# marzer/rt

Hardware: AMD Instinct MI355X
Metric: Mrays/s (W*H*spp per second) and wall-clock, 1920x1080x256spp scenes/basic.toml (higher is better)
Workload: dtype f32

## Files before the change

### rt_amd/csrc/context.hip

```cpp
#include "internal.hpp"

#include <algorithm>
#include <exception>
#include <new>

using namespace rt_hip;

namespace rt_hip
{
	namespace
	{
		thread_local std::string g_last_error;
	}

	rt_hip_status fail(rt_hip_status status, const char* format, ...)
	{
		char buffer[512];
		va_list args;
		va_start(args, format);
		std::vsnprintf(buffer, sizeof(buffer), format, args);
		va_end(args);
		g_last_error = buffer;
		return status;
	}
// ... 29 lines not shown
	return ok();
}

extern "C" rt_hip_status rt_hip_create(rt_hip_ctx** out_ctx, int device)
{
	if (!out_ctx)
		return fail(RT_HIP_INVALID_ARGUMENT, "rt_hip_create: out_ctx is NULL");
	*out_ctx = nullptr;
	int count = 0;
	if (hipGetDeviceCount(&count) != hipSuccess || count <= 0)
		return fail(RT_HIP_NO_DEVICE, "rt_hip_create: no HIP device is visible");
	if (device < 0 || device >= count)
		return fail(RT_HIP_NO_DEVICE, "rt_hip_create: device %d out of range (%d visible)", device, count);
	RT_HIP_TRY(hipSetDevice(device));
	hipDeviceProp_t props{};
	RT_HIP_TRY(hipGetDeviceProperties(&props, device));
	if (std::strncmp(props.gcnArchName, "gfx950", 6) != 0)
		return fail(RT_HIP_NO_DEVICE, "rt_hip_create: device %d is %s; this module is built for gfx950 only", device, props.gcnArchName);

	rt_hip_ctx* ctx = new (std::nothrow) rt_hip_ctx;
	if (!ctx)
		return fail(RT_HIP_RUNTIME_ERROR, "rt_hip_create: out of host memory");
	ctx->device = device;
	ctx->compute_units = props.multiProcessorCount > 0 ? static_cast<uint32_t>(props.multiProcessorCount) : 256u;
	ctx->workgroup_lds_bytes = props.sharedMemPerBlock;
	ctx->numa_node = numa_node_of(device);
	if (const char* knob = std::getenv("RT_HIP_NUMA_NODE"))
	{
		char* end = nullptr;
		const long v = std::strtol(knob, &end, 10);
		if (end != knob && v >= -1 && v < 1024)
			ctx->numa_node = static_cast<int>(v);
	}
	hipError_t e = ctx->counters.reserve(sizeof(device_counters));
	if (e == hipSuccess)
		e = hipEventCreate(&ctx->render_begin);
	if (e == hipSuccess)
		e = hipEventCreate(&ctx->render_end);
	if (e == hipSuccess)
		e = hipEventCreateWithFlags(&ctx->stripes_ready, hipEventDisableTiming);
	if (e == hipSuccess)
		e = hipEventCreateWithFlags(&ctx->counters_copied, hipEventDisableTiming);
	if (e == hipSuccess)
		e = hipEventCreate(&ctx->gathered);
	if (e == hipSuccess)
		e = hipEventCreate(&ctx->assembled);
	if (e == hipSuccess)
		e = hipEventCreate(&ctx->copied);
	if (e == hipSuccess)
		e = hipHostMalloc(reinterpret_cast<void**>(&ctx->counters_host), sizeof(device_counters), hipHostMallocDefault);
	if (e == hipSuccess)
		e = hipStreamCreateWithFlags(&ctx->stream, hipStreamNonBlocking);
	if (e != hipSuccess)
	{
		rt_hip_destroy(ctx);
		return fail(RT_HIP_RUNTIME_ERROR, "rt_hip_create: %s", hipGetErrorString(e));
	}
	*out_ctx = ctx;
	return ok();
}

extern "C" rt_hip_status rt_hip_create_multi(rt_hip_ctx** out_ctx, const int* devices, int n_devices, uint32_t multi_flags)
{
	if (!out_ctx)
		return fail(RT_HIP_INVALID_ARGUMENT, "rt_hip_create_multi: out_ctx is NULL");
	*out_ctx = nullptr;
// ... 401 lines not shown
```

### rt_amd/csrc/internal.hpp

```cpp
#pragma once

#include "../../include/rt_hip.h"
#include "contract.hpp"
#include "delivery.hpp"
#include "frame_group.hpp"
#include "kernels.hpp"
#include "progressive.hpp"
#include "adaptive.hpp"
#include "lights.hpp"

#include <rccl/rccl.h>

#include <atomic>
#include <chrono>
#include <condition_variable>
#include <cstdarg>
#include <cstdio>
#include <cstdlib>
#include <cstring>
#include <memory>
#include <mutex>
#include <string>
#include <thread>
#include <vector>

namespace rt_hip
{
	rt_hip_status fail(rt_hip_status status, const char* format, ...) __attribute__((format(printf, 2, 3)));
	const std::string& last_error();
	inline rt_hip_status ok() { return RT_HIP_OK; }

#define RT_HIP_TRY_NCCL(expr)                                                                                          \
	do                                                                                                                 \
	{                                                                                                                  \
		const ncclResult_t rt_hip_try_res = (expr);                                                                    \
		if (rt_hip_try_res != ncclSuccess)                                                                             \
			return ::rt_hip::fail(RT_HIP_RUNTIME_ERROR, "%s failed: %s", #expr, ncclGetErrorString(rt_hip_try_res));   \
	}                                                                                                                  \
	while (false)

#define RT_HIP_TRY(expr)                                                                                               \
	do                                                                                                                 \
// ... 219 lines not shown
	uint32_t box_bvh_count = 0;
	bool box_bvh_built = false;
	uint64_t box_bvh_sphere_stamp = 0;
	uint64_t box_bvh_builds = 0;
	size_t scene_bytes = 0;
	std::vector<float> emission;
	bool have_emission = false;
	uint32_t emission_rows = 0, emission_lights = 0;
	uint64_t emission_version = 0;
	rt_hip::device_buffer light_tables;
	uint64_t light_tables_uploads = 0, light_tables_version = 0;
	const float4* light_shading = nullptr;
	const uint32_t* light_scatter = nullptr;
	const float4* light_shading_sm = nullptr;
	const uint32_t* light_scatter_sm = nullptr;
	void* pinned_frame = nullptr;
	size_t pinned_bytes = 0;
	void* refused_frame = nullptr;
	size_t refused_bytes = 0;

	const void* asked_pointer = nullptr;
	bool asked_pointer_is_host = false;

	rt_hip_stats stats{};

	rt_hip::pass_state progressive;
	uint32_t progressive_passes = 0;
	rt_hip::device_buffer accum;
	std::vector<uint32_t> progressive_frame;
	rt_hip::denoise_state denoise;
	rt_hip::temporal_state temporal;
	rt_hip::adaptive_accumulation adaptive;

	rt_hip_ctx() = default;
	rt_hip_ctx(const rt_hip_ctx&) = delete;
	rt_hip_ctx& operator=(const rt_hip_ctx&) = delete;
};

namespace rt_hip
{
	rt_hip_ctx* member_of(rt_hip_ctx* ctx, int rank);

	struct scene_layout
	{
		size_t scx, scy, scz, sr, sm;
		size_t pnx, pny, pnz, pd, pm;
		size_t shading, type;
		size_t geometry, prim_shading, prim_metal;
		size_t prim_shading_sm, prim_scatter_sm;
		size_t box_bounds, albedo;
		size_t total;
	};
	struct scene_request
	{
		const rt_hip_scene* scene = nullptr;
		scene_layout layout{};
		uint64_t print = 0;
		bool indices_checked = false;
		const unsigned char* image = nullptr;
		small_scene small{}, small_sm{};
	};
	rt_hip_status open_request(scene_request& r, const rt_hip_scene* scene);
	rt_hip_status make_resident(rt_hip_ctx* ctx, scene_request& r);
	rt_hip_status ensure_bvh(rt_hip_ctx* ctx, bool device_build, hipStream_t stream, bool wait);
	rt_hip_status ensure_box_bvh(rt_hip_ctx* ctx, hipStream_t stream);
	rt_hip_status ensure_light_tables(rt_hip_ctx* ctx);

	struct render_pass
	{
		uint32_t first_sample, n_samples;
		float* d_accum;
		bool adaptive = false;
	};
	rt_hip_status render_device(rt_hip_ctx* ctx, uint32_t width, uint32_t height, uint64_t seed, uint32_t flags, const rt_hip_partition* part, uint32_t* d_rgba8, float* d_rgb_f32, void* stream, bool whole_frame_buffers, bool keep_stats, bool host_frame,
								const render_pass* pass = nullptr);
	rt_hip_status fetch_member_stats(rt_hip_ctx* ctx);
	rt_hip_stats stats_of_group_rank(const rt_hip_ctx* ctx, uint32_t rank);
	void sum_group_stats(const rt_hip_ctx* ctx, rt_hip_stats* out);

	constexpr uint32_t max_frame_side = 1u << 15;
	const char* refused_guide_flag(uint32_t flags);
	bool buffers_overlap(const void* a, size_t a_bytes, const void* b, size_t b_bytes);
	frame_params centre_frame_params(uint32_t width, uint32_t height, const float* matrix);
	rt_hip_status launch_guide(rt_hip_ctx* ctx, uint32_t width, uint32_t height, const float* matrix, bool trace_boxes, float* d_guide, hipStream_t stream);
	rt_hip_status launch_filter(rt_hip_ctx* ctx, uint32_t width, uint32_t height, const float* d_in, const float* d_guide, const rt_hip_denoise_params& params, float* d_out, uint32_t* d_rgba, hipStream_t stream);

	rt_hip_status render_multi(rt_hip_ctx* root, const rt_hip_scene* scene, uint32_t* pixels_rgba8888, uint32_t width, uint32_t height, uint64_t seed, uint32_t flags, float* rgb_f32, rt_hip_stats* stats, std::chrono::steady_clock::time_point entered);
	rt_hip_status render_group(rt_hip_ctx* ctx, const rt_hip_scene* scene, uint32_t* pixels_rgba8888, uint32_t width, uint32_t height, uint64_t seed, uint32_t flags, float* rgb_f32, rt_hip_stats* stats, std::chrono::steady_clock::time_point entered);

	int numa_node_of(int device);
	bool debug_frame();
	void place_stripes(void* ptr, size_t bytes, uint32_t width, uint32_t height, uint32_t stripe_rows, const std::vector<int>& node_of_rank);
	void unpin_frame(rt_hip_ctx* ctx);
	void track_frame_buffer(rt_hip_ctx* ctx, uint32_t* pixels, size_t bytes, bool pin, bool may_move_pages = true, const std::vector<int>* stripe_nodes = nullptr, uint32_t width = 0, uint32_t height = 0);
	uint32_t live_frame_locks();

	struct staging_frame
	{
		void* ptr = nullptr;
		size_t bytes = 0;
		bool registered = false;
		int view_device = -1;
		void* view = nullptr;
		hipError_t reserve(size_t wanted, int numa_node);
		void release();
		~staging_frame() { release(); }
		template <typename T>
		T* as() const
// ... 49 lines not shown
```

### rt_amd/csrc/kernels.hip

```cpp
#include "kernels.hpp"
#include "contract.hpp"
#include "scan.hpp"
#include "bvh_scan.hpp"
#include "box_bvh_scan.hpp"
#include "scan_streamed.hpp"
#include "handover.hpp"
#include "pixel_output.hpp"
#include "lane_state.hpp"
#include "queue_build.hpp"
#include "camera_forms.hpp"

#ifdef RT_HIP_FAST_BUILD
#define render_queue render_queue_fast
#define launch_render launch_render_fast
#endif

#include "../../include/rt_hip.h"

#include <algorithm>

#ifdef RT_HIP_REGION_COUNTERS
#define RT_HIP_REGION(i)                                                                                               \
	do                                                                                                                 \
	{                                                                                                                  \
// ... 54 lines not shown
			else if (RESIDENT)
			{
				for (uint32_t i = threadIdx.x; i < lds_spheres + s.n_planes; i += block_threads)
					lds[i] = s.primitive_geometry[(s.n_spheres - lds_spheres) + i];
			}
			if constexpr (BOXES && !BOXTREE)
			{
				for (uint32_t i = threadIdx.x; i < 2u * s.n_boxes; i += block_threads)
					lds_boxes[i] = s.box_bounds[i];
			}
			__syncthreads();

#ifdef RT_HIP_REGION_COUNTERS
			uint32_t region_runs[device_counters::regions] = {}, region_lanes[device_counters::regions] = {};
#endif
			const queue_words words = unpack_words<build>(q, item_sums, pixel_done);
			const uint32_t first_chunk = PASS ? words.first_chunk : 0u;
			float* const accum = PASS ? words.accum : nullptr;
			device_bvh bvh{};
			if constexpr (BVH)
				bvh = *words.bvh;
			device_box_bvh box_tree{};
			if constexpr (BOXTREE)
				box_tree = *words.box_tree;
			const uint32_t lane = threadIdx.x & 63u;
			const uint32_t wave = threadIdx.x >> 6;
			const uint32_t chunk_items = q.chunks << q.pixels_log2;
			const uint32_t items = HALF ? 2u * chunk_items : chunk_items;
			float* const slots = reinterpret_cast<float*>(lds + table_float4s) + static_cast<size_t>(wave) * chunk_items * slot_floats;
			const uint32_t tile_w = 1u << q.tile_w_log2;
			const uint32_t tile_h = (1u << q.pixels_log2) >> q.tile_w_log2;

			const uint32_t tile_x0 = (blockIdx.x * 4u + wave) * tile_w;
			const uint32_t tile_y0 = (gridDim.y - 1u - blockIdx.y) * tile_h;
			uint32_t next_item = 0;
			unsigned long long tile_stopped = 0;
			float* pass_sums = nullptr;
			if constexpr (ADAPT)
			{
				const adaptive_words adaptive = unpack_adaptive_words(accum, p);
				pass_sums = adaptive.pass_sums;
				const uint32_t lx = tile_x0 + (lane & (tile_w - 1u));
				const uint32_t ly = tile_y0 + (lane >> q.tile_w_log2);
				const bool in_frame = lane < (1u << q.pixels_log2) && lx < p.width && ly < p.local_rows;
				bool stopped = false;
				if (first_chunk && in_frame)
					stopped = (adaptive.pixel_state[static_cast<size_t>(output_row(ly, p)) * p.width + lx] & 0x80000000u) != 0u;
				tile_stopped = __builtin_amdgcn_ballot_w64(stopped);
				if ((__builtin_amdgcn_ballot_w64(in_frame) & ~tile_stopped) == 0)
					return;
			}

			const uint32_t items_per_pixel = (ROLLING && HALF) ? (p.samples_per_pixel + q.item_samples - 1u) / q.item_samples : q.chunks;
			const unsigned long long total_items = static_cast<unsigned long long>(p.width) * p.local_rows * items_per_pixel;
			unsigned long long block_next = 0, block_end = 0;
			unsigned long long prefetched = 0;
			uint32_t prefetched_count = ROLLING ? min(64u, q.lane_cap) : 64u;
			bool dry = false;
			if (ROLLING)
				prefetched = fetch_items(counters, prefetched_count);
#ifdef RT_HIP_WAVE_CLOCKS
			const unsigned long long clock_start = wall_clock64();
			unsigned long long clock_dry = 0;
#endif

			lane_state st;
			unsigned long long wave_segments = 0;
// ... 1006 lines not shown
		};

		queue_kernel select_kernel(const kernel_build& build)
		{
			if (build.scan > 0)
			{
				const int spheres = std::min(build.scan, static_cast<int>(scalar_max_spheres)), planes = std::min(build.planes, static_cast<int>(scalar_max_planes));
				for (const small_builds& known : small_kernels)
					if (known.spheres == spheres && known.planes == planes)
						return build.general_camera ? known.general_camera(build) : known.pinhole(build);
				return nullptr;
			}
			switch (build.scan)
			{
#ifndef RT_HIP_FAST_BUILD
				case scan_bvh: return table_of<scan_bvh>(build);
#endif
				case scan_resident:
					if (build.planes)
						return table_of<scan_resident, 1, false>(build);
					return build.general_camera ? table_of<scan_resident, 0, true>(build) : table_of<scan_resident, 0, false>(build);
				case scan_streamed_dense: return table_of<scan_streamed_dense>(build);
				case scan_streamed: return table_of<scan_streamed>(build);
				default: return table_of<scan_tiled>(build);
			}
		}

		struct kernel_words
		{
			queue_params queue;
			unsigned long long* item_sums;
			uint32_t* pixel_done;
		};
		kernel_words pack_words(const rolling_buffers& rolling, const launch_plan& plan)
		{
			const kernel_build& build = plan.build;
			kernel_words words = { plan.queue, rolling.item_sums, rolling.pixel_done };
			if (build.scan == scan_bvh)
				words.item_sums = reinterpret_cast<unsigned long long*>(const_cast<device_bvh*>(rolling.bvh));
#ifndef RT_HIP_FAST_BUILD
			if ((build.scan == scan_resident || build.scan == scan_bvh) && !build.boxes && !build.lights && (build.adaptive || build.pass))
			{
				words.queue.block_items = plan.first_chunk;
				words.pixel_done = reinterpret_cast<uint32_t*>(rolling.accum);
			}
#endif
			return words;
		}
	}

	uint32_t launch_render(const launch_arguments& a)
	{
		const launch_plan& plan = a.plan;
		if (plan.variant == RT_HIP_KERNEL_NONE)
			return RT_HIP_KERNEL_NONE;
		const queue_kernel kernel = select_kernel(plan.build);
		if (!kernel)
			return plan.variant;
		dim3 grid(plan.grid_x, plan.grid_y);
		if (scan_is_persistent(plan.build.scan))
		{
			launch_cache::entry& known = a.cache.persistent[plan.persistent_slot];
			if (known.lds_bytes != plan.lds_bytes || known.per_cu < 1)
			{
				int per_cu = 0;
				if (hipOccupancyMaxActiveBlocksPerMultiprocessor(&per_cu, kernel, static_cast<int>(block_threads), plan.lds_bytes) != hipSuccess || per_cu < 1)
					per_cu = 4;
				per_cu = std::min(per_cu, plan.per_cu_cap);
				(void)hipGetLastError();
				known.lds_bytes = plan.lds_bytes;
				known.per_cu = per_cu;
			}
			grid = dim3(std::min(grid.x, a.compute_units * static_cast<uint32_t>(known.per_cu)));
		}
		const kernel_words words = pack_words(a.rolling, plan);
		hipLaunchKernelGGL(kernel, grid, dim3(block_threads), plan.lds_bytes, a.stream, a.frame, words.queue, a.small, a.scene, a.scene.primitive_geometry, a.d_rgba8, a.d_rgb_f32, a.d_counters, words.item_sums, words.pixel_done);
		return plan.variant;
	}

#ifndef RT_HIP_FAST_BUILD
	void launch_preview(const frame_params& frame, const device_scene& scene, uint32_t* d_rgba8, float* d_rgb_f32, device_counters* d_counters, hipStream_t stream)
	{
		if (!frame.width || !frame.local_rows)
			return;
		const uint32_t rows_per_block = block_threads / 64u;
		const dim3 grid((frame.width + 63u) / 64u, (frame.local_rows + rows_per_block - 1u) / rows_per_block);
		hipLaunchKernelGGL(preview_frame, grid, dim3(block_threads), 0, stream, frame, scene, d_rgba8, d_rgb_f32, d_counters);
	}

	void launch_assemble(uint32_t width,
						 uint32_t height,
						 uint32_t world,
						 uint32_t stripe_rows,
						 uint32_t padded_local_rows,
						 const uint32_t* d_gathered,
						 uint32_t* d_frame,
						 uint32_t first_rank,
						 bool frame_is_host_memory,
						 hipStream_t stream)
	{
		const dim3 grid((width + block_threads - 1) / block_threads, height);
		if (frame_is_host_memory)
			hipLaunchKernelGGL(assemble_stripes<true>, grid, dim3(block_threads), 0, stream, width, height, world, stripe_rows, padded_local_rows, first_rank, d_gathered, d_frame);
		else
			hipLaunchKernelGGL(assemble_stripes<false>, grid, dim3(block_threads), 0, stream, width, height, world, stripe_rows, padded_local_rows, first_rank, d_gathered, d_frame);
	}

#endif
// ... 2 lines not shown
```

### rt_amd/csrc/kernels.hpp

```cpp
#pragma once

#include <hip/hip_runtime.h>
#include <stdint.h>
#include "launch_plan.hpp"
#include "frame_setup.hpp"

namespace rt_hip
{
	struct device_bvh
	{
		const float4* nodes;
		const float4* spheres;
		const uint32_t* order;
		const uint32_t* always;
		uint32_t root, n_tree, n_always;
		float cx, cy, cz, radius;
	};

	struct device_scene
	{
		uint32_t n_spheres, n_planes, n_materials;
		const float* sphere_cx;
		const float* sphere_cy;
		const float* sphere_cz;
// ... 51 lines not shown
#endif
#ifdef RT_HIP_BVH_CHECK
		unsigned long long bvh_checked, bvh_disagreements;
#endif
#ifdef RT_HIP_WAVE_CLOCKS
		static constexpr unsigned clocked_waves = 16384;
		unsigned long long wave_clocks[clocked_waves][3];
#endif
	};

	struct launch_cache
	{
		struct entry
		{
			size_t lds_bytes = 0;
			int per_cu = 0;
		};
		entry persistent[persistent_cache_slots];
	};

	struct launch_arguments
	{
		const frame_params& frame;
		const device_scene& scene;
		const small_scene& small;
		const launch_plan& plan;
		uint32_t* d_rgba8;
		float* d_rgb_f32;
		device_counters* d_counters;
		const rolling_buffers& rolling;
		uint32_t compute_units;
		launch_cache& cache;
		hipStream_t stream;
	};

	uint32_t launch_render(const launch_arguments& a);

	uint32_t launch_render_fast(const launch_arguments& a);

	void launch_preview(const frame_params& frame, const device_scene& scene, uint32_t* d_rgba8, float* d_rgb_f32, device_counters* d_counters, hipStream_t stream);

	void launch_assemble(uint32_t width,
						 uint32_t height,
						 uint32_t world,
						 uint32_t stripe_rows,
						 uint32_t padded_local_rows,
						 const uint32_t* d_gathered,
						 uint32_t* d_frame,
						 uint32_t first_rank,
						 bool frame_is_host_memory,
						 hipStream_t stream);
}
```

### rt_amd/csrc/render.hip

```cpp
#include "internal.hpp"

#include <algorithm>
#include <cstdio>
#include <exception>

using namespace rt_hip;

namespace
{
	bool is_host_memory(rt_hip_ctx* ctx, const void* pointer)
	{
		if (pointer != ctx->asked_pointer)
		{
			hipPointerAttribute_t attributes{};
			const hipError_t e = hipPointerGetAttributes(&attributes, pointer);
			if (e != hipSuccess)
				(void)hipGetLastError();
			ctx->asked_pointer = pointer;
			ctx->asked_pointer_is_host = e == hipSuccess && attributes.type == hipMemoryTypeHost;
		}
		return ctx->asked_pointer_is_host;
	}
}

extern "C" rt_hip_status rt_hip_render_device(rt_hip_ctx* ctx,
											  uint32_t width,
											  uint32_t height,
											  uint64_t seed,
											  uint32_t flags,
											  const rt_hip_partition* part,
											  uint32_t* d_rgba8,
											  float* d_rgb_f32,
											  void* stream)
{
	return render_device(ctx, width, height, seed, flags, part, d_rgba8, d_rgb_f32, stream, false, true, ctx && d_rgba8 && is_host_memory(ctx, d_rgba8));
}

extern "C" rt_hip_status rt_hip_render_pass_device(rt_hip_ctx* ctx,
													   uint32_t width,
													   uint32_t height,
													   uint64_t seed,
													   uint32_t flags,
													   const rt_hip_partition* part,
													   uint32_t first_sample,
													   uint32_t n_samples,
													   float* d_accum,
													   uint32_t* d_rgba8,
													   float* d_rgb_f32,
													   void* stream)
{
	if (first_sample % sample_chunk)
		return fail(RT_HIP_INVALID_ARGUMENT, "rt_hip_render_pass_device: first_sample %u is not a multiple of %u (a pass continues the chunk-wise fold of the pixel sums)", first_sample, sample_chunk);
	if (!ctx || !d_accum || !d_rgba8)
		return fail(RT_HIP_INVALID_ARGUMENT, "rt_hip_render_pass_device: NULL argument");
	if (const char* const refused = refused_pass_flag(flags))
		return fail(RT_HIP_UNSUPPORTED, "rt_hip_render_pass_device: %s is not available for passes (0x%x): they take RT_HIP_FLAG_SM_MATERIALS, RT_HIP_FLAG_BVH, RT_HIP_FLAG_BVH_DEVICE_BUILD and RT_HIP_FLAG_STATS", refused, flags);
	if (!ctx->have_scene)
		return fail(RT_HIP_NO_SCENE, "rt_hip_render_pass_device: no scene uploaded");
	const uint32_t total = ctx->samples_per_pixel;
	if (total > pass_max_samples_per_pixel)
		return fail(RT_HIP_UNSUPPORTED, "rt_hip_render_pass_device: %u samples per pixel: the samples' random windows alias beyond %u", total, pass_max_samples_per_pixel);
	if (!n_samples || first_sample >= total || n_samples > total - first_sample || (n_samples % sample_chunk && first_sample + n_samples != total))
		return fail(RT_HIP_INVALID_ARGUMENT, "rt_hip_render_pass_device: samples [%u, %u + %u) are not whole chunks of %u within the scene's %u samples per pixel (the last pass alone may end on the sample count)", first_sample,
					first_sample, n_samples, sample_chunk, total);
	const render_pass pass = { first_sample, n_samples, d_accum };
	return render_device(ctx, width, height, seed, flags & pass_flag_mask, part, d_rgba8, d_rgb_f32, stream, false, true, is_host_memory(ctx, d_rgba8), &pass);
}

namespace rt_hip
{
rt_hip_status render_device(rt_hip_ctx* ctx, uint32_t width, uint32_t height, uint64_t seed, uint32_t flags, const rt_hip_partition* part, uint32_t* d_rgba8, float* d_rgb_f32, void* stream, bool whole_frame_buffers, bool keep_stats, bool host_frame,
							const render_pass* pass)
{
	if (!ctx || !d_rgba8)
		return fail(RT_HIP_INVALID_ARGUMENT, "rt_hip_render_device: NULL argument");
	const render_check checked = check_render_request(width, height, flags, part);
	if (checked.status)
		return fail(checked.status, "%s", checked.message);
	flags = checked.flags;
	if (!ctx->have_scene)
		return fail(RT_HIP_NO_SCENE, "rt_hip_render_device: no scene uploaded");
	if (flags & RT_HIP_FLAG_EMISSION)
	{
		const light_check table = check_emission_table("rt_hip_render_device", ctx->have_emission, ctx->emission_rows, ctx->scene.n_materials);
		if (table.status)
			return fail(table.status, "%s", table.message);
	}
	RT_HIP_TRY(hipSetDevice(ctx->device));
	const hipStream_t s = static_cast<hipStream_t>(stream);
	if (ctx->launched && ctx->last_stream != s)
		RT_HIP_TRY(hipStreamSynchronize(ctx->last_stream));

	frame_request wanted{};
	wanted.width = width, wanted.height = height, wanted.partition = checked.partition;
	wanted.samples_per_pixel = pass ? pass->first_sample + pass->n_samples : ctx->samples_per_pixel, wanted.max_bounces = ctx->max_bounces;
	wanted.seed = seed, wanted.whole_frame_buffers = whole_frame_buffers;
	std::copy(ctx->inverse_view_projection, ctx->inverse_view_projection + 16, wanted.inverse_view_projection);
	const frame_params f = make_frame_params(wanted);

	launch_plan plan{};
	rolling_buffers rolling;
	if (!(flags & RT_HIP_FLAG_PREVIEW))
	{
		launch_request request{};
		request.n_spheres = ctx->scene.n_spheres, request.n_planes = ctx->scene.n_planes, request.planes_tame = ctx->scene.planes_tame != 0;
		request.width = width, request.local_rows = f.local_rows, request.samples_per_pixel = pass ? ctx->samples_per_pixel : f.samples_per_pixel;
		if (pass)
			request.pass_first_sample = pass->first_sample, request.pass_samples = pass->n_samples, request.adaptive = pass->adaptive;
		request.camera = camera_form_of(f);
		request.flags = flags, request.host_frame = host_frame, request.fast_arithmetic = (flags & RT_HIP_FLAG_FAST) != 0;
		request.n_boxes = ctx->scene.n_boxes;
		request.n_lights = (flags & RT_HIP_FLAG_EMISSION) ? ctx->emission_lights : 0u;
		request.lds_limit = ctx->workgroup_lds_bytes;
		plan = plan_launch(request);
		if (plan.refusal[0])
			return fail(RT_HIP_UNSUPPORTED, "rt_hip_render_device: %s", plan.refusal);
		if (pass && plan.slot_bytes > max_slot_bytes)
			return fail(RT_HIP_UNSUPPORTED, "rt_hip_render_pass_device: a pass of %u samples is more than the kernels hold chunk sums for (4096 per pass; the frame's samples_per_pixel has no such limit)", pass->n_samples);
		if (plan.slot_bytes > max_slot_bytes)
			return fail(RT_HIP_UNSUPPORTED, "rt_hip_render_device: %u samples per pixel are more than the kernels hold chunk sums for (4096; the reference clamps to 1000, src/scene.cpp:544)", f.samples_per_pixel);
		if (plan.build.scan == scan_bvh)
		{
			if (const rt_hip_status st = ensure_bvh(ctx, (flags & RT_HIP_FLAG_BVH) ? checked.bvh_device_build : false, s, keep_stats))
				return st;
			RT_HIP_TRY(hipSetDevice(ctx->device));
			rolling.bvh = ctx->bvh_descriptor;
		}
		if (plan.build.box_tree)
		{
			if (const rt_hip_status st = ensure_box_bvh(ctx, s))
				return st;
			rolling.bvh = ctx->box_bvh_block.as<const device_bvh>();
		}
		if (pass)
			rolling.accum = pass->d_accum;
		if (plan.build.lights)
		{
			if (const rt_hip_status st = ensure_light_tables(ctx))
				return st;
			RT_HIP_TRY(hipSetDevice(ctx->device));
		}
		if (plan.item_sums_bytes > ctx->item_sums.bytes && plan.queue.halves && plan.big_scene && ctx->item_sums.reserve(plan.item_sums_bytes) != hipSuccess)
		{
			(void)hipGetLastError();
			request.flags |= RT_HIP_FLAG_FORCE_WHOLE_CHUNKS;
			request.flags &= ~static_cast<uint32_t>(RT_HIP_FLAG_FORCE_HALF_CHUNKS);
			plan = plan_launch(request);
		}
		if (plan.item_sums_bytes > (64ull << 30))
			return fail(RT_HIP_UNSUPPORTED, "%s: %ux%u at %u samples per pixel needs %zu GiB for the chunk sums of a scene of this size", pass ? "rt_hip_render_pass_device" : "rt_hip_render_device", width, height, f.samples_per_pixel, plan.item_sums_bytes >> 30);
		if (plan.item_sums_bytes)
		{
			RT_HIP_TRY(ctx->item_sums.reserve(plan.item_sums_bytes));
			RT_HIP_TRY(ctx->pixel_done.reserve(plan.pixel_done_bytes));
			RT_HIP_TRY(hipMemsetAsync(ctx->pixel_done.ptr, 0, plan.pixel_done_bytes, s));
			rolling.item_sums = ctx->item_sums.as<unsigned long long>();
			rolling.pixel_done = ctx->pixel_done.as<uint32_t>();
		}
	}
	device_counters* const counters = ctx->counters.as<device_counters>();
	if (keep_stats)
	{
		RT_HIP_TRY(hipMemsetAsync(counters, 0, sizeof(device_counters), s));
		RT_HIP_TRY(hipEventRecord(ctx->render_begin, s));
	}
	else if (plan.big_scene)
		RT_HIP_TRY(hipMemsetAsync(&counters->next_item, 0, sizeof(counters->next_item), s));
	uint32_t variant = RT_HIP_KERNEL_PREVIEW;
	if (flags & RT_HIP_FLAG_PREVIEW)
		launch_preview(f, ctx->scene, d_rgba8, d_rgb_f32, counters, s);
	else if (flags & RT_HIP_FLAG_FAST)
		variant = launch_render_fast({ f, ctx->scene, ctx->small, plan, d_rgba8, d_rgb_f32, counters, rolling, ctx->compute_units, ctx->cache, s });
	else if (plan.build.lights)
	{
		device_scene lit = ctx->scene;
		lit.primitive_shading = ctx->light_shading, lit.primitive_scatter = ctx->light_scatter;
		lit.primitive_shading_sm = ctx->light_shading_sm, lit.primitive_scatter_sm = ctx->light_scatter_sm;
		variant = launch_render({ f, lit, (flags & RT_HIP_FLAG_SM_MATERIALS) ? ctx->small_sm : ctx->small, plan, d_rgba8, d_rgb_f32, counters, rolling, ctx->compute_units, ctx->cache, s });
	}
	else
		variant = launch_render({ f, ctx->scene, (flags & RT_HIP_FLAG_SM_MATERIALS) ? ctx->small_sm : ctx->small, plan, d_rgba8, d_rgb_f32, counters, rolling, ctx->compute_units, ctx->cache, s });
	RT_HIP_TRY(hipGetLastError());
	ctx->launched = true;
	ctx->last_stream = s;
	if (keep_stats)
	{
		RT_HIP_TRY(hipEventRecord(ctx->render_end, s));
		RT_HIP_TRY(hipMemcpyAsync(ctx->counters_host, counters, sizeof(device_counters), hipMemcpyDeviceToHost, s));
		RT_HIP_TRY(hipEventRecord(ctx->counters_copied, s));
	}
	ctx->render_recorded = keep_stats;
	ctx->stats.kernel_variant = variant;
	ctx->stats.primary_samples = static_cast<uint64_t>(f.local_rows) * width * ((flags & RT_HIP_FLAG_PREVIEW) ? 1u : (pass ? pass->n_samples : f.samples_per_pixel));
	if (!keep_stats)
	{
		ctx->stats.render_ms = 0.0f;
		ctx->stats.segments = ctx->stats.sphere_tests = ctx->stats.plane_tests = 0;
	}
	return ok();
}
}

extern "C" rt_hip_status rt_hip_assemble_device(rt_hip_ctx* ctx,
												uint32_t width,
												uint32_t height,
												uint32_t world,
												uint32_t stripe_rows,
												const uint32_t* d_gathered,
												uint32_t* d_frame,
												void* stream)
{
	if (!ctx || !d_gathered || !d_frame)
		return fail(RT_HIP_INVALID_ARGUMENT, "rt_hip_assemble_device: NULL argument");
	if (!width || !height || !world || !stripe_rows)
// ... 175 lines not shown
			return fail(RT_HIP_RUNTIME_ERROR, "rt_hip_render: out of host memory");
		struct abandon_unless_finished
		{
			frame_delivery* delivery;
			~abandon_unless_finished()
			{
				if (delivery)
					delivery->abandon();
			}
		} staged{ nullptr };
		struct drain_before_abandoning
		{
			hipStream_t stream;
			bool armed;
			~drain_before_abandoning()
			{
				if (armed && hipStreamSynchronize(stream) != hipSuccess)
					(void)hipGetLastError();
			}
		} drain{ ctx->stream, false };
		if (!d_frame)
		{
			if (const rt_hip_status st = delivery->begin(pixels_rgba8888, pixels, &d_frame))
				return st;
			staged.delivery = delivery;
		}
		const size_t rgb_bytes = pixels * 3 * sizeof(float);
		if (rgb_f32)
		{
			RT_HIP_TRY(ctx->frame_rgb.reserve(rgb_bytes));
			RT_HIP_TRY(ctx->staging_rgb.reserve(rgb_bytes));
		}
		drain.armed = true;
		if (const rt_hip_status st = render_device(ctx, width, height, seed, flags & render_flag_mask, nullptr, d_frame, rgb_f32 ? ctx->frame_rgb.as<float>() : nullptr, ctx->stream, false, keep_stats, true))
			return st;
		if (staged.delivery)
			staged.delivery->launched();
		hipError_t e = hipSuccess;
		if (rgb_f32)
			e = hipMemcpyAsync(ctx->staging_rgb.ptr, ctx->frame_rgb.ptr, rgb_bytes, hipMemcpyDeviceToHost, ctx->stream);
		const auto issued = std::chrono::steady_clock::now();
		if (e == hipSuccess && keep_stats)
			e = hipEventSynchronize(ctx->render_end);
		const auto t0 = std::chrono::steady_clock::now();
		const hipError_t drained = hipStreamSynchronize(ctx->stream);
		drain.armed = drained != hipSuccess;
		RT_HIP_TRY(e);
		RT_HIP_TRY(drained);
		if (staged.delivery)
		{
			staged.delivery->finish();
			ctx->phases.carrier_bands = static_cast<uint32_t>(staged.delivery->carrier.bands());
			ctx->phases.carrier_bands_early = static_cast<uint32_t>(staged.delivery->carrier.early_bands());
			ctx->phases.carrier_helpers = staged.delivery->carrier.helpers();
			staged.delivery = nullptr;
		}
		if (rgb_f32)
			delivery->carrier.copy(rgb_f32, ctx->staging_rgb.ptr, rgb_bytes);
		ctx->stats.readback_ms = keep_stats ? static_cast<float>(seconds_since(t0) * 1e3) : 0.0f;
		ctx->phases.host_issue_ms = static_cast<float>(std::chrono::duration<double>(issued - entered).count() * 1e3);
		ctx->phases.host_wait_ms = static_cast<float>(seconds_since(issued) * 1e3);
		if (keep_stats)
			ctx->phases.render_ms = elapsed_or_zero(ctx->render_begin, ctx->render_end);
		if (stats)
			return rt_hip_stats_fetch(ctx, stats);
		return ok();
	}
// ... 6 lines not shown
```

### rt_amd/csrc/scene.hip

```cpp
#include "internal.hpp"
#include "bvh.hpp"
#include "box_bvh.hpp"
#include "box_bvh_scan.hpp"
#include "bvh_build.hpp"
#include "bvh_build_device.hpp"

#include <algorithm>
#include <cmath>
#include <cstring>
#include <exception>

using namespace rt_hip;

namespace
{
	rt_hip_status check_scene_pointers(const rt_hip_scene& s)
	{
		if (!s.samples_per_pixel || !s.max_bounces)
			return fail(RT_HIP_INVALID_ARGUMENT, "scene: samples_per_pixel and max_bounces must be >= 1");
		if (s.n_spheres && (!s.sphere_center_x || !s.sphere_center_y || !s.sphere_center_z || !s.sphere_radius || !s.sphere_material))
			return fail(RT_HIP_INVALID_ARGUMENT, "scene: %u spheres but a sphere column is NULL", s.n_spheres);
		if (s.n_planes && (!s.plane_normal_x || !s.plane_normal_y || !s.plane_normal_z || !s.plane_d || !s.plane_material))
			return fail(RT_HIP_INVALID_ARGUMENT, "scene: %u planes but a plane column is NULL", s.n_planes);
		if (!s.n_materials && (s.n_spheres || s.n_planes || s.n_boxes))
// ... 228 lines not shown
		const auto t0 = std::chrono::steady_clock::now();
		const rt_hip_scene& s = *r.scene;
		const scene_layout& L = r.layout;
		RT_HIP_TRY(hipSetDevice(ctx->device));
		const bool resident = ctx->have_scene && ctx->scene_fingerprint == r.print && ctx->scene_bytes == L.total && ctx->scene_columns.bytes >= L.total;
		if (!resident)
		{
			if (!r.indices_checked)
			{
				if (const rt_hip_status st = check_scene_indices(s))
					return st;
				r.indices_checked = true;
			}
			if (!r.image)
				if (const rt_hip_status st = build_image(ctx, r))
					return st;
			RT_HIP_TRY(hipDeviceSynchronize());
			ctx->have_scene = false;
			RT_HIP_TRY(ctx->scene_columns.reserve(L.total));
			RT_HIP_TRY(hipMemcpy(ctx->scene_columns.ptr, r.image, L.total, hipMemcpyHostToDevice));
			ctx->scene_fingerprint = r.print;
			ctx->scene_bytes = L.total;
			ctx->scene_uploads++;
			uint64_t box_print = 0xcbf29ce484222325ull ^ s.n_boxes;
			for (size_t k = 0; k < static_cast<size_t>(s.n_boxes) * 8u; k++)
			{
				uint32_t word;
				std::memcpy(&word, r.image + L.box_bounds + k * 4u, 4);
				box_print = (box_print ^ word) * 0x100000001b3ull;
			}
			ctx->box_columns_print = box_print;
			ctx->small = r.small;
			ctx->small_sm = r.small_sm;

			unsigned char* base = ctx->scene_columns.as<unsigned char>();
			device_scene& d = ctx->scene;
			d.n_spheres = s.n_spheres;
			d.n_planes = s.n_planes;
			d.n_materials = s.n_materials;
			d.sphere_cx = reinterpret_cast<const float*>(base + L.scx);
			d.sphere_cy = reinterpret_cast<const float*>(base + L.scy);
			d.sphere_cz = reinterpret_cast<const float*>(base + L.scz);
			d.sphere_r = reinterpret_cast<const float*>(base + L.sr);
			d.sphere_material = reinterpret_cast<const uint32_t*>(base + L.sm);
			d.plane_nx = reinterpret_cast<const float*>(base + L.pnx);
			d.plane_ny = reinterpret_cast<const float*>(base + L.pny);
			d.plane_nz = reinterpret_cast<const float*>(base + L.pnz);
			d.plane_d = reinterpret_cast<const float*>(base + L.pd);
			d.plane_material = reinterpret_cast<const uint32_t*>(base + L.pm);
			d.material_shading = reinterpret_cast<const float4*>(base + L.shading);
			d.material_type = reinterpret_cast<const uint32_t*>(base + L.type);
			d.primitive_geometry = reinterpret_cast<const float4*>(base + L.geometry);
			d.primitive_shading = reinterpret_cast<const float4*>(base + L.prim_shading);
			d.primitive_scatter = reinterpret_cast<const uint32_t*>(base + L.prim_metal);
			d.primitive_shading_sm = reinterpret_cast<const float4*>(base + L.prim_shading_sm);
			d.primitive_scatter_sm = reinterpret_cast<const uint32_t*>(base + L.prim_scatter_sm);
			d.n_boxes = s.n_boxes;
			d.box_bounds = reinterpret_cast<const float4*>(base + L.box_bounds);
			d.material_albedo = reinterpret_cast<const float4*>(base + L.albedo);
			d.planes_tame = 1u;
			for (uint32_t k = 0; k < s.n_planes; k++)
				for (const float n : { s.plane_normal_x[k], s.plane_normal_y[k], s.plane_normal_z[k] })
					if (!(std::fabs(n) <= 0x1p40f))
						d.planes_tame = 0u;
		}
		ctx->samples_per_pixel = s.samples_per_pixel;
// ... 244 lines not shown
```

Measured before the change: 241,800.

## Render provably sky-only top rows with a cheap sky-band kernel

On the host, a conservative geometric test over the pinhole ray field and a small sphere table finds how many top rows can never hit any sphere, when the scene has no planes. Those rows go to a dedicated kernel that only evaluates camera jitter and the sky colour per sample. The main render kernel is launched over the remaining rows through a row offset in the queue word. This drops the intersection loop for rows whose result is only sky, at the cost of host-side analysis (cached per frame and scene) and an extra kernel launch. Any error in the conservative bound would give wrong pixels.

Result: faster. 268,900 (median of 6 runs) (+11.2%).

```diff
diff --git a/rt_amd/csrc/context.hip b/rt_amd/csrc/context.hip
--- a/rt_amd/csrc/context.hip
+++ b/rt_amd/csrc/context.hip
@@ -85,6 +85,10 @@
 		if (end != knob && v >= -1 && v < 1024)
 			ctx->numa_node = static_cast<int>(v);
 	}
+	if (const char* knob = std::getenv("RT_HIP_SKY_BAND"))
+		ctx->sky_band_enabled = std::strcmp(knob, "0") != 0;
+	if (const char* knob = std::getenv("RT_HIP_SKY_BAND_LOG"))
+		ctx->sky_band_log = std::strcmp(knob, "1") == 0;
 	hipError_t e = ctx->counters.reserve(sizeof(device_counters));
 	if (e == hipSuccess)
 		e = hipEventCreate(&ctx->render_begin);
diff --git a/rt_amd/csrc/internal.hpp b/rt_amd/csrc/internal.hpp
--- a/rt_amd/csrc/internal.hpp
+++ b/rt_amd/csrc/internal.hpp
@@ -8,6 +8,7 @@
 #include "progressive.hpp"
 #include "adaptive.hpp"
 #include "lights.hpp"
+#include "sky_band.hpp"
 
 #include <rccl/rccl.h>
 
@@ -293,6 +294,19 @@
 	rt_hip::temporal_state temporal;
 	rt_hip::adaptive_accumulation adaptive;
 
+	bool sky_band_enabled = true;
+	bool sky_band_log = false;
+	std::vector<float> sphere_table;
+	struct
+	{
+		bool valid = false;
+		uint64_t scene_uploads = 0;
+		uint32_t flags = 0;
+		int scan = 0;
+		rt_hip::frame_params frame{};
+		uint32_t rows = 0;
+	} sky_band_asked;
+
 	rt_hip_ctx() = default;
 	rt_hip_ctx(const rt_hip_ctx&) = delete;
 	rt_hip_ctx& operator=(const rt_hip_ctx&) = delete;
@@ -334,7 +348,7 @@
 		bool adaptive = false;
 	};
 	rt_hip_status render_device(rt_hip_ctx* ctx, uint32_t width, uint32_t height, uint64_t seed, uint32_t flags, const rt_hip_partition* part, uint32_t* d_rgba8, float* d_rgb_f32, void* stream, bool whole_frame_buffers, bool keep_stats, bool host_frame,
-								const render_pass* pass = nullptr);
+								const render_pass* pass = nullptr, bool sky_band = false);
 	rt_hip_status fetch_member_stats(rt_hip_ctx* ctx);
 	rt_hip_stats stats_of_group_rank(const rt_hip_ctx* ctx, uint32_t rank);
 	void sum_group_stats(const rt_hip_ctx* ctx, rt_hip_stats* out);
diff --git a/rt_amd/csrc/kernels.hip b/rt_amd/csrc/kernels.hip
--- a/rt_amd/csrc/kernels.hip
+++ b/rt_amd/csrc/kernels.hip
@@ -110,7 +110,7 @@
 			const uint32_t tile_h = (1u << q.pixels_log2) >> q.tile_w_log2;
 
 			const uint32_t tile_x0 = (blockIdx.x * 4u + wave) * tile_w;
-			const uint32_t tile_y0 = (gridDim.y - 1u - blockIdx.y) * tile_h;
+			const uint32_t tile_y0 = (gridDim.y - 1u - blockIdx.y) * tile_h + ((!ROLLING && !PASS) ? q.block_items : 0u);
 			uint32_t next_item = 0;
 			unsigned long long tile_stopped = 0;
 			float* pass_sums = nullptr;
@@ -1183,10 +1183,12 @@
 			unsigned long long* item_sums;
 			uint32_t* pixel_done;
 		};
-		kernel_words pack_words(const rolling_buffers& rolling, const launch_plan& plan)
+		kernel_words pack_words(const rolling_buffers& rolling, const launch_plan& plan, uint32_t first_row)
 		{
 			const kernel_build& build = plan.build;
 			kernel_words words = { plan.queue, rolling.item_sums, rolling.pixel_done };
+			if (!scan_is_persistent(build.scan))
+				words.queue.block_items = first_row;
 			if (build.scan == scan_bvh)
 				words.item_sums = reinterpret_cast<unsigned long long*>(const_cast<device_bvh*>(rolling.bvh));
 #ifndef RT_HIP_FAST_BUILD
@@ -1224,7 +1226,7 @@
 			}
 			grid = dim3(std::min(grid.x, a.compute_units * static_cast<uint32_t>(known.per_cu)));
 		}
-		const kernel_words words = pack_words(a.rolling, plan);
+		const kernel_words words = pack_words(a.rolling, plan, a.first_row);
 		hipLaunchKernelGGL(kernel, grid, dim3(block_threads), plan.lds_bytes, a.stream, a.frame, words.queue, a.small, a.scene, a.scene.primitive_geometry, a.d_rgba8, a.d_rgb_f32, a.d_counters, words.item_sums, words.pixel_done);
 		return plan.variant;
 	}
diff --git a/rt_amd/csrc/kernels.hpp b/rt_amd/csrc/kernels.hpp
--- a/rt_amd/csrc/kernels.hpp
+++ b/rt_amd/csrc/kernels.hpp
@@ -107,11 +107,14 @@
 		uint32_t compute_units;
 		launch_cache& cache;
 		hipStream_t stream;
+		uint32_t first_row = 0;
 	};
 
 	uint32_t launch_render(const launch_arguments& a);
 
 	uint32_t launch_render_fast(const launch_arguments& a);
+
+	void launch_sky_band(const frame_params& band, uint32_t* d_rgba8, float* d_rgb_f32, device_counters* d_counters, hipStream_t stream);
 
 	void launch_preview(const frame_params& frame, const device_scene& scene, uint32_t* d_rgba8, float* d_rgb_f32, device_counters* d_counters, hipStream_t stream);
 
diff --git a/rt_amd/csrc/render.hip b/rt_amd/csrc/render.hip
--- a/rt_amd/csrc/render.hip
+++ b/rt_amd/csrc/render.hip
@@ -33,7 +33,7 @@
 											  float* d_rgb_f32,
 											  void* stream)
 {
-	return render_device(ctx, width, height, seed, flags, part, d_rgba8, d_rgb_f32, stream, false, true, ctx && d_rgba8 && is_host_memory(ctx, d_rgba8));
+	return render_device(ctx, width, height, seed, flags, part, d_rgba8, d_rgb_f32, stream, false, true, ctx && d_rgba8 && is_host_memory(ctx, d_rgba8), nullptr, true);
 }
 
 extern "C" rt_hip_status rt_hip_render_pass_device(rt_hip_ctx* ctx,
@@ -70,7 +70,7 @@
 namespace rt_hip
 {
 rt_hip_status render_device(rt_hip_ctx* ctx, uint32_t width, uint32_t height, uint64_t seed, uint32_t flags, const rt_hip_partition* part, uint32_t* d_rgba8, float* d_rgb_f32, void* stream, bool whole_frame_buffers, bool keep_stats, bool host_frame,
-							const render_pass* pass)
+							const render_pass* pass, bool sky_band)
 {
 	if (!ctx || !d_rgba8)
 		return fail(RT_HIP_INVALID_ARGUMENT, "rt_hip_render_device: NULL argument");
@@ -100,6 +100,7 @@
 
 	launch_plan plan{};
 	rolling_buffers rolling;
+	uint32_t band_rows = 0, band_variant = RT_HIP_KERNEL_NONE;
 	if (!(flags & RT_HIP_FLAG_PREVIEW))
 	{
 		launch_request request{};
@@ -157,6 +158,32 @@
 			rolling.item_sums = ctx->item_sums.as<unsigned long long>();
 			rolling.pixel_done = ctx->pixel_done.as<uint32_t>();
 		}
+		if (ctx->sky_band_enabled && sky_band && !pass)
+		{
+			frame_params asked = f;
+			asked.frame_key_a = asked.frame_key_b = 0u;
+			auto& last = ctx->sky_band_asked;
+			if (!(last.valid && last.scene_uploads == ctx->scene_uploads && last.flags == flags && last.scan == plan.build.scan && std::memcmp(&last.frame, &asked, sizeof(asked)) == 0))
+			{
+				const sky_band_request rule = { ctx->sphere_table.data(), ctx->scene.n_spheres, ctx->scene.n_planes, flags, false, false, plan.build.scan, &f };
+				last.rows = sky_band_rows(rule);
+				last.valid = true, last.scene_uploads = ctx->scene_uploads, last.flags = flags, last.scan = plan.build.scan, last.frame = asked;
+			}
+			if (last.rows)
+			{
+				request.local_rows = f.local_rows - last.rows;
+				const launch_plan below = plan_launch(request);
+				const bool tile_per_wave = below.build.scan > 0 || below.build.scan == scan_resident;
+				if (!below.refusal[0] && below.slot_bytes <= max_slot_bytes && !below.item_sums_bytes && tile_per_wave)
+				{
+					band_rows = last.rows;
+					band_variant = plan.variant;
+					plan = below;
+				}
+			}
+		}
+		if (ctx->sky_band_log)
+			std::fprintf(stderr, "rt_hip sky band: rows %u of %u (%ux%u, flags 0x%x)\n", band_rows, height, width, height, flags);
 	}
 	device_counters* const counters = ctx->counters.as<device_counters>();
 	if (keep_stats)
@@ -167,6 +194,16 @@
 	else if (plan.big_scene)
 		RT_HIP_TRY(hipMemsetAsync(&counters->next_item, 0, sizeof(counters->next_item), s));
 	uint32_t variant = RT_HIP_KERNEL_PREVIEW;
+	const auto launch_band = [&]()
+	{
+		frame_params band = f;
+		band.local_rows = band_rows;
+		launch_sky_band(band, d_rgba8, d_rgb_f32, counters, s);
+	};
+#ifndef RT_HIP_SKY_BAND_LAST
+	if (band_rows)
+		launch_band();
+#endif
 	if (flags & RT_HIP_FLAG_PREVIEW)
 		launch_preview(f, ctx->scene, d_rgba8, d_rgb_f32, counters, s);
 	else if (flags & RT_HIP_FLAG_FAST)
@@ -179,7 +216,13 @@
 		variant = launch_render({ f, lit, (flags & RT_HIP_FLAG_SM_MATERIALS) ? ctx->small_sm : ctx->small, plan, d_rgba8, d_rgb_f32, counters, rolling, ctx->compute_units, ctx->cache, s });
 	}
 	else
-		variant = launch_render({ f, ctx->scene, (flags & RT_HIP_FLAG_SM_MATERIALS) ? ctx->small_sm : ctx->small, plan, d_rgba8, d_rgb_f32, counters, rolling, ctx->compute_units, ctx->cache, s });
+		variant = launch_render({ f, ctx->scene, (flags & RT_HIP_FLAG_SM_MATERIALS) ? ctx->small_sm : ctx->small, plan, d_rgba8, d_rgb_f32, counters, rolling, ctx->compute_units, ctx->cache, s, band_rows });
+#ifdef RT_HIP_SKY_BAND_LAST
+	if (band_rows)
+		launch_band();
+#endif
+	if (band_rows)
+		variant = band_variant;
 	RT_HIP_TRY(hipGetLastError());
 	ctx->launched = true;
 	ctx->last_stream = s;
@@ -421,7 +464,7 @@
 			RT_HIP_TRY(ctx->staging_rgb.reserve(rgb_bytes));
 		}
 		drain.armed = true;
-		if (const rt_hip_status st = render_device(ctx, width, height, seed, flags & render_flag_mask, nullptr, d_frame, rgb_f32 ? ctx->frame_rgb.as<float>() : nullptr, ctx->stream, false, keep_stats, true))
+		if (const rt_hip_status st = render_device(ctx, width, height, seed, flags & render_flag_mask, nullptr, d_frame, rgb_f32 ? ctx->frame_rgb.as<float>() : nullptr, ctx->stream, false, keep_stats, true, nullptr, true))
 			return st;
 		if (staged.delivery)
 			staged.delivery->launched();
diff --git a/rt_amd/csrc/scene.hip b/rt_amd/csrc/scene.hip
--- a/rt_amd/csrc/scene.hip
+++ b/rt_amd/csrc/scene.hip
@@ -284,6 +284,13 @@
 			ctx->box_columns_print = box_print;
 			ctx->small = r.small;
 			ctx->small_sm = r.small_sm;
+			ctx->sphere_table.clear();
+			if (s.n_spheres <= sky_band_max_spheres)
+			{
+				ctx->sphere_table.resize(static_cast<size_t>(s.n_spheres) * 4u);
+				if (s.n_spheres)
+					std::memcpy(ctx->sphere_table.data(), r.image + L.geometry, ctx->sphere_table.size() * sizeof(float));
+			}
 
 			unsigned char* base = ctx->scene_columns.as<unsigned char>();
 			device_scene& d = ctx->scene;
diff --git a/rt_amd/csrc/sky_band.cpp b/rt_amd/csrc/sky_band.cpp
--- /dev/null
+++ b/rt_amd/csrc/sky_band.cpp
@@ -0,0 +1,206 @@
+#include "sky_band.hpp"
+
+#include <cmath>
+#include <initializer_list>
+
+namespace rt_hip
+{
+	namespace
+	{
+		struct ray_field
+		{
+			double d0[3], d1[3], d2[3];
+			double g00, g01, g02, g11, g12, g22;
+			double det, inv_det, inv_g11, inv_g22;
+		};
+
+		double length2_at(const ray_field& f, double u, double v)
+		{
+			return f.g00 + u * (2.0 * f.g01 + u * f.g11) + v * (2.0 * f.g02 + v * f.g22) + 2.0 * u * v * f.g12;
+		}
+
+		double lesser(double a, double b) { return b < a ? b : a; }
+		double greater(double a, double b) { return b > a ? b : a; }
+		double clamp_to(double x, double lo, double hi) { return x < lo ? lo : (x > hi ? hi : x); }
+
+		double least_length2(const ray_field& f, double u0, double u1, double v0, double v1)
+		{
+			const double u = (f.g12 * f.g02 - f.g22 * f.g01) * f.inv_det, v = (f.g12 * f.g01 - f.g11 * f.g02) * f.inv_det;
+			if (u >= u0 && u <= u1 && v >= v0 && v <= v1)
+				return length2_at(f, u, v);
+			double least = INFINITY;
+			for (const double fixed_u : { u0, u1 })
+				least = lesser(least, length2_at(f, fixed_u, clamp_to(-(f.g02 + fixed_u * f.g12) * f.inv_g22, v0, v1)));
+			for (const double fixed_v : { v0, v1 })
+				least = lesser(least, length2_at(f, clamp_to(-(f.g01 + fixed_v * f.g12) * f.inv_g11, u0, u1), fixed_v));
+			return least;
+		}
+
+		struct sphere_terms
+		{
+			double q0, q1, q2;
+			double w2, r2, m;
+			double w_length;
+			bool pierces;
+			double u_pierce, v_pierce;
+		};
+
+		bool certainly_missed(const ray_field& f, const sphere_terms& s, uint32_t x0, uint32_t x1, uint32_t y0, uint32_t y1)
+		{
+			const double u0 = static_cast<double>(x0) - 1.0, u1 = static_cast<double>(x1) + 1.0, v0 = static_cast<double>(y0) - 1.0, v1 = static_cast<double>(y1) + 1.0;
+			double q_min = INFINITY, q_max = -INFINITY, t2_max = 0.0, t2_corner[4];
+			for (int corner = 0; corner < 4; corner++)
+			{
+				const double u = (corner & 1) ? u1 : u0, v = (corner & 2) ? v1 : v0;
+				const double q = s.q0 + s.q1 * u + s.q2 * v;
+				q_min = lesser(q_min, q), q_max = greater(q_max, q);
+				t2_corner[corner] = length2_at(f, u, v);
+				t2_max = greater(t2_max, t2_corner[corner]);
+			}
+			const double t2_min = least_length2(f, u0, u1, v0, v1);
+			if (!(t2_min > 0.0))
+				return false;
+			const double scale = s.w2 + s.r2 + t2_max + s.m * s.m * (1.0 / 64.0);
+			const double room = sky_band_epsilon * scale;
+			const double q2_max = greater(q_min * q_min, q_max * q_max);
+			if (s.w2 - q2_max / t2_min - s.r2 >= room)
+				return true;
+			const double t_max = std::sqrt(t2_max);
+			const double behind = sky_band_epsilon * (s.w_length + t_max + s.m * 0.125) * t_max;
+			if (s.w2 - 2.0 * q_max + t2_min - s.r2 >= room && q_max - t2_min <= -behind)
+				return true;
+			if (s.pierces && s.u_pierce >= u0 && s.u_pierce <= u1 && s.v_pierce >= v0 && s.v_pierce <= v1)
+				return false;
+			double ratio_max = q2_max / t2_max;
+			for (int corner = 0; corner < 4; corner++)
+			{
+				const double u = (corner & 1) ? u1 : u0, v = (corner & 2) ? v1 : v0;
+				const double q = s.q0 + s.q1 * u + s.q2 * v;
+				ratio_max = greater(ratio_max, q * q / t2_corner[corner]);
+			}
+			for (int edge = 0; edge < 4; edge++)
+			{
+				const bool along_v = edge < 2;
+				const double fixed = along_v ? (edge ? u1 : u0) : (edge == 3 ? v1 : v0);
+				const double t0 = along_v ? v0 : u0, t1 = along_v ? v1 : u1;
+				const double a = along_v ? f.g00 + fixed * (2.0 * f.g01 + fixed * f.g11) : f.g00 + fixed * (2.0 * f.g02 + fixed * f.g22);
+				const double b = along_v ? f.g02 + fixed * f.g12 : f.g01 + fixed * f.g12;
+				const double c = along_v ? f.g22 : f.g11;
+				const double k0 = along_v ? s.q0 + s.q1 * fixed : s.q0 + s.q2 * fixed, k1 = along_v ? s.q2 : s.q1;
+				const double den = k1 * b - k0 * c;
+				if (den != 0.0)
+				{
+					const double t = -(k1 * a - k0 * b) / den;
+					if (t > t0 && t < t1)
+					{
+						const double q = k0 + k1 * t;
+						ratio_max = greater(ratio_max, q * q / (a + t * (2.0 * b + t * c)));
+					}
+				}
+			}
+			return s.w2 - ratio_max - s.r2 >= room;
+		}
+
+		bool strip_is_clear(const ray_field& f, const sphere_terms& s, uint32_t x0, uint32_t x1, uint32_t y0, uint32_t y1, bool asked = false)
+		{
+			if (!asked && certainly_missed(f, s, x0, x1, y0, y1))
+				return true;
+			const uint32_t columns = x1 - x0, rows = y1 - y0;
+			const bool narrow = columns <= sky_band_cell_columns;
+			if (rows > 1u && (narrow || rows * 32u >= columns))
+			{
+				const uint32_t middle = y0 + rows / 2u;
+				return strip_is_clear(f, s, x0, x1, middle, y1) && strip_is_clear(f, s, x0, x1, y0, middle);
+			}
+			if (narrow)
+				return false;
+			const uint32_t middle = x0 + columns / 2u;
+			return strip_is_clear(f, s, x0, middle, y0, y1) && strip_is_clear(f, s, middle, x1, y0, y1);
+		}
+
+		uint32_t first_doubtful_row(const ray_field& f, const sphere_terms& s, uint32_t x0, uint32_t x1, uint32_t y0, uint32_t y1)
+		{
+			if (y0 >= y1 || certainly_missed(f, s, x0, x1, y0, y1))
+				return y1;
+			const uint32_t columns = x1 - x0, strips = (y1 - y0) / sky_band_strip_rows;
+			if (strips <= 1u)
+				return strip_is_clear(f, s, x0, x1, y0, y1, true) ? y1 : y0;
+			if (columns <= sky_band_cell_columns || (y1 - y0) * 4u >= columns)
+			{
+				const uint32_t middle = y0 + (strips / 2u) * sky_band_strip_rows;
+				const uint32_t upper = first_doubtful_row(f, s, x0, x1, y0, middle);
+				return upper < middle ? upper : first_doubtful_row(f, s, x0, x1, middle, y1);
+			}
+			const uint32_t middle = x0 + columns / 2u;
+			const uint32_t left = first_doubtful_row(f, s, x0, middle, y0, y1);
+			return left == y0 ? y0 : first_doubtful_row(f, s, middle, x1, y0, left);
+		}
+	}
+
+	uint32_t sky_band_rows(const sky_band_request& request)
+	{
+		if (!request.frame || request.pass || request.adaptive || (request.flags & sky_band_excluded_flags) || request.n_planes != 0u)
+			return 0u;
+		if (!(request.scan > 0 || request.scan == scan_resident) || request.n_spheres > sky_band_max_spheres || (request.n_spheres && !request.spheres))
+			return 0u;
+		const frame_params& p = *request.frame;
+		if (p.world != 1u || p.rank != 0u || p.local_rows != p.height || !p.pinhole)
+			return 0u;
+		if (!p.width || p.width > sky_band_max_side || p.height > sky_band_max_side || p.height < sky_band_strip_rows)
+			return 0u;
+		if (!p.samples_per_pixel || p.samples_per_pixel >= (1u << 20) || !p.max_bounces)
+			return 0u;
+
+		ray_field f{};
+		double eye[3], eye2 = 0.0;
+		for (int c = 0; c < 3; c++)
+		{
+			f.d0[c] = p.ray_d0[c], f.d1[c] = p.ray_d1[c], f.d2[c] = p.ray_d2[c];
+			eye[c] = p.ray_eye[c];
+			eye2 += eye[c] * eye[c];
+			if (!(static_cast<double>(p.ray_j1[c]) * 0x1.0p24 == f.d1[c]) || !(static_cast<double>(p.ray_j2[c]) * 0x1.0p24 == f.d2[c]))
+				return 0u;
+			f.g00 += f.d0[c] * f.d0[c], f.g01 += f.d0[c] * f.d1[c], f.g02 += f.d0[c] * f.d2[c];
+			f.g11 += f.d1[c] * f.d1[c], f.g12 += f.d1[c] * f.d2[c], f.g22 += f.d2[c] * f.d2[c];
+		}
+		f.det = f.g11 * f.g22 - f.g12 * f.g12;
+		f.inv_det = 1.0 / f.det, f.inv_g11 = 1.0 / f.g11, f.inv_g22 = 1.0 / f.g22;
+		if (!(f.g00 < INFINITY) || !(eye2 < INFINITY) || !(f.g11 > 0.0) || !(f.g22 > 0.0) || !(f.det > 0x1.0p-20 * f.g11 * f.g22) || !(f.det < INFINITY))
+			return 0u;
+
+		uint32_t rows = (p.height / sky_band_strip_rows) * sky_band_strip_rows;
+		for (uint32_t i = 0; i < request.n_spheres && rows; i++)
+		{
+			const float* const sphere = request.spheres + 4u * static_cast<size_t>(i);
+			sphere_terms s{};
+			double c2 = 0.0;
+			for (int c = 0; c < 3; c++)
+			{
+				const double centre = sphere[c], w = centre - eye[c];
+				c2 += centre * centre;
+				s.w2 += w * w;
+				s.q0 += w * f.d0[c], s.q1 += w * f.d1[c], s.q2 += w * f.d2[c];
+			}
+			s.r2 = sphere[3];
+			s.m = std::sqrt(eye2) + std::sqrt(c2);
+			s.w_length = std::sqrt(s.w2);
+			const double n[3] = { f.d1[1] * f.d2[2] - f.d1[2] * f.d2[1], f.d1[2] * f.d2[0] - f.d1[0] * f.d2[2], f.d1[0] * f.d2[1] - f.d1[1] * f.d2[0] };
+			double wn = 0.0, d0n = 0.0;
+			for (int c = 0; c < 3; c++)
+				wn += (static_cast<double>(sphere[c]) - eye[c]) * n[c], d0n += f.d0[c] * n[c];
+			s.pierces = false;
+			if (wn != 0.0)
+			{
+				const double lambda = d0n / wn, right1 = lambda * s.q1 - f.g01, right2 = lambda * s.q2 - f.g02;
+				s.u_pierce = (f.g22 * right1 - f.g12 * right2) * f.inv_det, s.v_pierce = (f.g11 * right2 - f.g12 * right1) * f.inv_det;
+				s.pierces = true;
+				if (!(s.u_pierce > -INFINITY && s.u_pierce < INFINITY && s.v_pierce > -INFINITY && s.v_pierce < INFINITY))
+					return 0u;
+			}
+			if (!(c2 < INFINITY) || !(s.w2 < INFINITY) || !(s.r2 >= 0.0) || !(s.r2 < INFINITY))
+				return 0u;
+			rows = first_doubtful_row(f, s, 0u, p.width, 0u, rows);
+		}
+		return rows;
+	}
+}
diff --git a/rt_amd/csrc/sky_band.hip b/rt_amd/csrc/sky_band.hip
--- /dev/null
+++ b/rt_amd/csrc/sky_band.hip
@@ -0,0 +1,88 @@
+#include "kernels.hpp"
+#include "contract.hpp"
+#include "pixel_output.hpp"
+#include "lane_state.hpp"
+#include "camera_forms.hpp"
+
+namespace rt_hip
+{
+	namespace
+	{
+		struct pinhole_build
+		{
+			static constexpr bool PINHOLE_ONLY = true, EYE_ONLY = false, NEVER_PINHOLE = false;
+		};
+
+		constexpr uint32_t band_pixels = 64;
+
+		__global__ __launch_bounds__(block_threads) void sky_band_rows_kernel(const frame_params p, const uint32_t chunks, uint32_t* __restrict__ out_rgba, float* __restrict__ out_rgb, device_counters* __restrict__ counters)
+		{
+			__shared__ float sums[block_threads / 64u][3][band_pixels];
+			const uint32_t lane = threadIdx.x & 63u, wave = threadIdx.x >> 6;
+			const uint32_t lx = blockIdx.x * band_pixels + lane, ly = blockIdx.y;
+			const uint32_t gy = global_row(ly, p);
+			lane_state st;
+			camera_base<pinhole_build>(st, p, static_cast<float>(lx), static_cast<float>(gy));
+			st.keys.function_key = pixel_function_key(p.frame_key_a, gy * p.width + lx);
+			st.keys.stride = pixel_stride(p.frame_key_b, st.keys.function_key);
+			vec3 colour = { 0.0f, 0.0f, 0.0f };
+			for (uint32_t first_chunk = 0; first_chunk < chunks; first_chunk += block_threads / 64u)
+			{
+				const uint32_t chunk = first_chunk + wave;
+				if (chunk < chunks)
+				{
+					const uint32_t first = chunk * sample_chunk, end = min(first + sample_chunk, p.samples_per_pixel);
+					st.chunk_sum = { 0.0f, 0.0f, 0.0f };
+					st.window = sample_counter(st.keys.stride, first);
+					st.window_end = sample_counter(st.keys.stride, end);
+					do
+					{
+						st.counter = st.window + st.keys.stride;
+						const uint32_t word = step_word_at(st.counter, st.keys);
+						float jx = step_numerator(word * step_mul_a), jy = step_numerator(word * step_mul_b);
+						if (st.window == 0u)
+							jx = jy = 0x1.0p23f;
+						const vec3 toward = { fma(p.ray_j1[0], jx, fma(p.ray_j2[0], jy, st.base_x)), fma(p.ray_j1[1], jx, fma(p.ray_j2[1], jy, st.base_y)),
+											  fma(p.ray_j1[2], jx, fma(p.ray_j2[2], jy, st.base_z)) };
+						const float inv = inv_sqrt_rn(dot(toward, toward));
+						const float dir_y = toward.y * inv;
+						st.throughput = { 1.0f, 1.0f, 1.0f };
+						st.chunk_sum = st.chunk_sum + st.throughput * sky(dir_y);
+						st.window += st.keys.stride << draws_per_sample_log2;
+					}
+					while (st.window != st.window_end);
+					sums[wave][0][lane] = st.chunk_sum.x;
+					sums[wave][1][lane] = st.chunk_sum.y;
+					sums[wave][2][lane] = st.chunk_sum.z;
+				}
+				__syncthreads();
+				if (wave == 0u)
+				{
+					const uint32_t parked = min(chunks - first_chunk, block_threads / 64u);
+					for (uint32_t k = 0; k < parked; k++)
+					{
+						const vec3 sum = { sums[k][0][lane], sums[k][1][lane], sums[k][2][lane] };
+						colour = (first_chunk + k) ? colour + sum : sum;
+					}
+				}
+				__syncthreads();
+			}
+			if (wave == 0u && lx < p.width)
+				finish_pixel(colour, p, lx, ly, out_rgba, out_rgb);
+			if (threadIdx.x == 0u)
+			{
+				const uint32_t pixels = min(band_pixels, p.width - blockIdx.x * band_pixels);
+				atomicAdd(&counters->segments[(blockIdx.x + blockIdx.y * 7u) % device_counters::segment_counters], static_cast<unsigned long long>(pixels) * p.samples_per_pixel);
+			}
+		}
+	}
+
+	void launch_sky_band(const frame_params& band, uint32_t* d_rgba8, float* d_rgb_f32, device_counters* d_counters, hipStream_t stream)
+	{
+		if (!band.width || !band.local_rows || !band.samples_per_pixel)
+			return;
+		const uint32_t chunks = (band.samples_per_pixel + sample_chunk - 1u) / sample_chunk;
+		const dim3 grid((band.width + band_pixels - 1u) / band_pixels, band.local_rows);
+		hipLaunchKernelGGL(sky_band_rows_kernel, grid, dim3(block_threads), 0, stream, band, chunks, d_rgba8, d_rgb_f32, d_counters);
+	}
+}
diff --git a/rt_amd/csrc/sky_band.hpp b/rt_amd/csrc/sky_band.hpp
--- /dev/null
+++ b/rt_amd/csrc/sky_band.hpp
@@ -0,0 +1,30 @@
+#pragma once
+
+#include <stdint.h>
+#include "../../include/rt_hip.h"
+#include "frame_setup.hpp"
+#include "launch_plan.hpp"
+
+namespace rt_hip
+{
+	constexpr uint32_t sky_band_strip_rows = 8;
+	constexpr uint32_t sky_band_cell_columns = 64;
+	constexpr uint32_t sky_band_max_spheres = 64;
+	constexpr uint32_t sky_band_max_side = 1u << 15;
+
+	constexpr double sky_band_epsilon = 0x1.0p-12;
+
+	constexpr uint32_t sky_band_excluded_flags = RT_HIP_FLAG_FAST | RT_HIP_FLAG_PREVIEW | RT_HIP_FLAG_TRACE_BOXES | RT_HIP_FLAG_BOX_BVH | RT_HIP_FLAG_EMISSION | RT_HIP_FLAG_BVH | RT_HIP_FLAG_SM_MATERIALS;
+
+	struct sky_band_request
+	{
+		const float* spheres;
+		uint32_t n_spheres, n_planes;
+		uint32_t flags;
+		bool pass, adaptive;
+		int scan;
+		const frame_params* frame;
+	};
+
+	uint32_t sky_band_rows(const sky_band_request& request);
+}
```
